# ClashLuke/LocAtE

Measured on AMD Instinct MI355X. Metric: images/sec (G+D step) 64x64 bs=64, higher is better.
Workload: dtype f32 (contractions fp32-faithful on the matrix cores: 2 x scaled fp16 operand pieces / 3 MFMAs per slice where the operand's largest magnitude comes with it, else 3 x bf16 pieces / 6 MFMAs; fp32 accumulate); 1 GPU; LocAtE G+D step, 64x64 RGB, batch 64 per GPU (the fp32 variant - the reference's own precision - of BASELINE.json configs[1]: 64x64 RGB bs 64), self/feature attention at 16x16 and 64x64, random-init weights; global_batch=64, image_size=64, parallelism=dp1, launch=hipGraph replay, G-step generator pass on a second stream

## Files before the change

include/locate_hip.h:

```cpp
#ifndef LOCATE_HIP_H
#define LOCATE_HIP_H
#include <stddef.h>
#include <stdint.h>
#ifdef __cplusplus
extern "C" {
#endif

const char* locate_last_error(void);
int locate_abi_version(void);
int locate_device_info(char* arch_name, int name_len, int* cu_count, int* wave_size);

int locate_roottanh_fwd(const float* x, float* y, int64_t n, void* absmax , void* stream);
int locate_absmax_words(void);
int locate_roottanh_bwd(const float* x, const float* gy, float* gx, int64_t n, int accumulate, void* absmax, void* stream);
int locate_absmax(const float* x, int64_t n, void* absmax, void* stream);
int locate_act_cat_rows_fwd(const float* latent, const float* pre, float* out, int rows, int z, int w, void* stream);
int locate_act_rows_bwd(const float* pre, const float* g, int64_t g_row_stride, const float* g_add, float* gpre, int rows, int w,
                        void* stream);
int locate_add3(const float* a, int64_t a_bs, const float* b, int64_t b_bs, const float* c, int64_t c_bs, float* out, int batch,
                int64_t per, void* stream);
int locate_tanh_fwd(const float* x, float* y, int64_t n, void* stream);
int locate_tanh_bwd(const float* y, const float* gy, float* gx, int64_t n, void* stream);

size_t locate_norm_stats_workspace_bytes(void);
// ... 32 lines not shown
int locate_pool2_upsample2x_fwd(const float* x, float* y, int64_t planes, int H, int W, void* stream);
int locate_pool2_upsample2x_bwd(const float* gy, float* gx, int64_t planes, int H, int W, int accumulate, void* stream);
int locate_avgpool2_fwd(const float* x, float* y, int64_t planes, int H, int W, void* stream);
int locate_avgpool2_bwd(const float* gy, float* gx, int64_t planes, int H, int W, int accumulate, void* stream);
int locate_feature_pool_fwd(const float* x, float* y, int64_t n_out, int r, void* stream);
int locate_feature_pool_bwd(const float* gy, float* gx, int64_t n_out, int r, int accumulate, void* stream);
int locate_copy_channels(const float* src, float* dst, int B, int C, int hw, int64_t src_batch_stride,
                         int64_t dst_batch_stride, int accumulate, void* stream);

size_t locate_sn_workspace_bytes(int h, int wd);
int locate_sn_power_iter(const float* w, float* u, float* v, float* sigma, float* wv, int h, int wd, void* workspace,
                         void* stream);
size_t locate_sn_table_record_bytes(void);
int locate_sn_power_iter_batched(const void* table, int n_layers, int max_h, int max_wd, void* stream);
int locate_sn_weight_bwd(const double* inner_partial, int n_partial, const float* u, const float* v, const float* sigma,
                         const float* wv, float* gw, float* du, float* dsigma_out, int h, int wd, void* stream);
size_t locate_sn_group_workspace_bytes(void);
int locate_sn_weight_bwd_grouped(const float* gy, int64_t gy_bs, const float* y, int64_t y_bs, const float* bias, int groups,
                                 int Bg, int M, int plane, const float* sigma_tab, int sigma_stride, const float* u,
                                 const float* v, const float* wv, int64_t wv_stride, float* gw, float* du,
                                 float* dsigma_total_out, int h, int wd, void* workspace, void* stream);
int locate_sn_dv_batched(const void* table, int n_layers, int max_h, int max_wd, void* stream);

size_t locate_conv_panel_bytes(const int* geom, int adjoint);
int locate_conv_pack_panel(const int* geom, int adjoint, const float* w, float* panel, void* stream);
size_t locate_conv_pack_job_bytes(void);
int locate_conv_pack_job(const int* geom, int adjoint, const float* w, float* panel, int block_start, void* job_out,
                         int* blocks_out, int direct, const void* weight_absmax);
int locate_conv_pack_panels(const void* jobs, int n_jobs, int total_blocks, int any_f16, int passes, void* stream);
int locate_conv_pack_job_is_direct(const void* job);
int locate_conv_pack_job_is_window(const void* job);
int locate_conv_win_ok(const int* geom, int adjoint_fmt, int64_t x_bs, const void* x);
size_t locate_conv_win_workspace_bytes(const int* geom, int adjoint_fmt);
size_t locate_conv_fwd_workspace_bytes(const int* geom);
size_t locate_conv_counter_bytes(void);
int locate_conv_fwd(const int* geom, const float* x, int64_t x_bs, const float* panel, const float* scale,
                    int scale_group_batch, int scale_stride, const float* bias, float* y, int64_t y_bs, void* workspace,
                    void* counters, int precision, const void* x_absmax, const void* act_epilogue, void* stream);
size_t locate_conv_dgrad_workspace_bytes(const int* geom);
int locate_conv_dgrad(const int* geom, const float* gy, int64_t gy_bs, const float* panel, const float* scale,
                      int scale_group_batch, int scale_stride, const float* bias, float* gx, int64_t gx_bs, void* workspace,
                      void* counters, int precision, const void* gy_absmax, const void* act_epilogue, void* stream);
size_t locate_conv_wgrad_workspace_bytes(const int* geom);
int locate_conv_wgrad_partials(const int* geom);
int locate_conv_wgrad(const int* geom, const float* x, int64_t x_bs, const float* gy, int64_t gy_bs, float* gw,
                      const float* w_ref, const float* inv_scale, int scale_group_batch, int scale_stride,
                      double* inner_partial, void* workspace, int precision, const void* x_absmax, const void* gy_absmax,
                      void* deferred_reduce, void* stream);
int locate_conv_wgrad_group_partials(const int* geom, int groups);
size_t locate_conv_wgrad_group_workspace_bytes(const int* geom, int groups);
size_t locate_slab_reduce_record_bytes(void);
int locate_slab_reduce_max(void);
int locate_slab_reduce_record_blocks(const void* record);
int locate_slab_reduce_batch(const void* records, int n, void* stream);

size_t locate_wgrad_batch_record_bytes(void);
int locate_wgrad_batch_max(void);
int locate_wgrad_batch_record(const int* geom, const float* x, int64_t x_bs, const float* gy, int64_t gy_bs, float* gw,
                              const float* w_ref, const float* inv_scale, int scale_group_batch, int scale_stride,
                              double* inner_partial, void* record);
int locate_wgrad_batch(const void* records, int n, void* stream);

int locate_dwconv_fwd(const int* geom, const float* x, int64_t x_bs, const float* w, const float* scale, int scale_group_batch,
                      int scale_stride, float* y, int64_t y_bs, void* stream);
int locate_dwconv_dgrad(const int* geom, const float* gy, int64_t gy_bs, const float* w, const float* scale,
                        int scale_group_batch, int scale_stride, float* gx, int64_t gx_bs, void* stream);
// ... 82 lines not shown
```

locate_amd/_lib.py:

```python
import ctypes
import os

import torch

_HERE = os.path.dirname(os.path.abspath(__file__))
LIB_PATH = os.path.join(_HERE, "csrc", "liblocate_hip_dbg.so" if os.environ.get("LOCATE_HIP_DEBUG_LIBRARY") == "1"
                        else "liblocate_hip.so")

c_p = ctypes.c_void_p
c_i = ctypes.c_int
c_i64 = ctypes.c_int64
c_f = ctypes.c_float
c_d = ctypes.c_double
c_sz = ctypes.c_size_t
c_ip = ctypes.POINTER(ctypes.c_int)

PROTOTYPES = {
    "locate_last_error": (ctypes.c_char_p, []),
    "locate_abi_version": (c_i, []),
    "locate_device_info": (c_i, [ctypes.c_char_p, c_i, c_ip, c_ip]),
    "locate_roottanh_fwd": (c_i, [c_p, c_p, c_i64, c_p, c_p]),
    "locate_roottanh_bwd": (c_i, [c_p, c_p, c_p, c_i64, c_i, c_p, c_p]),
    "locate_act_cat_rows_fwd": (c_i, [c_p, c_p, c_p, c_i, c_i, c_i, c_p]),
    "locate_act_rows_bwd": (c_i, [c_p, c_p, c_i64, c_p, c_p, c_i, c_i, c_p]),
# ... 20 lines not shown
    "locate_gate_fwd": (c_i, [c_p, c_p, c_i, c_p, c_p, c_i64, c_i, c_p]),
    "locate_gate_fwd_stats": (c_i, [c_p, c_p, c_i, c_p, c_p, c_i64, c_i, c_i, c_p, c_p]),
    "locate_gate_bwd_workspace_bytes": (c_sz, [c_i64]),
    "locate_gate_bwd": (c_i, [c_p, c_p, c_i, c_p, c_p, c_p, c_p, c_p, c_i64, c_i, c_p, c_i, c_p, c_p]),
    "locate_softmax_fwd": (c_i, [c_p, c_p, c_i64, c_i, c_p]),
    "locate_softmax_bwd": (c_i, [c_p, c_p, c_p, c_i64, c_i, c_p]),
    "locate_upsample2x_fwd": (c_i, [c_p, c_p, c_i64, c_i, c_i, c_p]),
    "locate_upsample2x_bwd": (c_i, [c_p, c_p, c_i64, c_i, c_i, c_p]),
    "locate_pool2_upsample2x_fwd": (c_i, [c_p, c_p, c_i64, c_i, c_i, c_p]),
    "locate_pool2_upsample2x_bwd": (c_i, [c_p, c_p, c_i64, c_i, c_i, c_i, c_p]),
    "locate_avgpool2_fwd": (c_i, [c_p, c_p, c_i64, c_i, c_i, c_p]),
    "locate_avgpool2_bwd": (c_i, [c_p, c_p, c_i64, c_i, c_i, c_i, c_p]),
    "locate_feature_pool_fwd": (c_i, [c_p, c_p, c_i64, c_i, c_p]),
    "locate_feature_pool_bwd": (c_i, [c_p, c_p, c_i64, c_i, c_i, c_p]),
    "locate_copy_channels": (c_i, [c_p, c_p, c_i, c_i, c_i, c_i64, c_i64, c_i, c_p]),
    "locate_sn_workspace_bytes": (c_sz, [c_i, c_i]),
    "locate_sn_power_iter": (c_i, [c_p, c_p, c_p, c_p, c_p, c_i, c_i, c_p, c_p]),
    "locate_sn_table_record_bytes": (c_sz, []),
    "locate_sn_power_iter_batched": (c_i, [c_p, c_i, c_i, c_i, c_p]),
    "locate_sn_weight_bwd": (c_i, [c_p, c_i, c_p, c_p, c_p, c_p, c_p, c_p, c_p, c_i, c_i, c_p]),
    "locate_sn_group_workspace_bytes": (c_sz, []),
    "locate_sn_weight_bwd_grouped": (c_i, [c_p, c_i64, c_p, c_i64, c_p, c_i, c_i, c_i, c_i, c_p, c_i, c_p, c_p, c_p, c_i64, c_p,
                                           c_p, c_p, c_i, c_i, c_p, c_p]),
    "locate_sn_dv_batched": (c_i, [c_p, c_i, c_i, c_i, c_p]),
    "locate_conv_panel_bytes": (c_sz, [c_ip, c_i]),
    "locate_conv_pack_panel": (c_i, [c_ip, c_i, c_p, c_p, c_p]),
    "locate_conv_pack_job_bytes": (c_sz, []),
    "locate_conv_pack_job": (c_i, [c_ip, c_i, c_p, c_p, c_i, c_p, c_ip, c_i, c_p]),
    "locate_conv_pack_panels": (c_i, [c_p, c_i, c_i, c_i, c_i, c_p]),
    "locate_conv_pack_job_is_direct": (c_i, [c_p]),
    "locate_conv_pack_job_is_window": (c_i, [c_p]),
    "locate_conv_win_ok": (c_i, [c_ip, c_i, c_i64, c_p]),
    "locate_conv_win_workspace_bytes": (c_sz, [c_ip, c_i]),
    "locate_conv_fwd_workspace_bytes": (c_sz, [c_ip]),
    "locate_conv_counter_bytes": (c_sz, []),
    "locate_conv_fwd": (c_i, [c_ip, c_p, c_i64, c_p, c_p, c_i, c_i, c_p, c_p, c_i64, c_p, c_p, c_i, c_p, c_p, c_p]),
    "locate_conv_dgrad_workspace_bytes": (c_sz, [c_ip]),
    "locate_conv_dgrad": (c_i, [c_ip, c_p, c_i64, c_p, c_p, c_i, c_i, c_p, c_p, c_i64, c_p, c_p, c_i, c_p, c_p, c_p]),
    "locate_conv_wgrad_workspace_bytes": (c_sz, [c_ip]),
    "locate_conv_wgrad_partials": (c_i, [c_ip]),
    "locate_conv_wgrad": (c_i, [c_ip, c_p, c_i64, c_p, c_i64, c_p, c_p, c_p, c_i, c_i, c_p, c_p, c_i, c_p, c_p, c_p, c_p]),
    "locate_conv_wgrad_group_partials": (c_i, [c_ip, c_i]),
    "locate_conv_wgrad_group_workspace_bytes": (c_sz, [c_ip, c_i]),
    "locate_slab_reduce_record_bytes": (c_sz, []),
    "locate_slab_reduce_max": (c_i, []),
    "locate_slab_reduce_record_blocks": (c_i, [c_p]),
    "locate_slab_reduce_batch": (c_i, [c_p, c_i, c_p]),
    "locate_dwconv_fwd": (c_i, [c_ip, c_p, c_i64, c_p, c_p, c_i, c_i, c_p, c_i64, c_p]),
    "locate_dwconv_dgrad": (c_i, [c_ip, c_p, c_i64, c_p, c_p, c_i, c_i, c_p, c_i64, c_p]),
    "locate_dwconv_wgrad_workspace_bytes": (c_sz, [c_ip]),
    "locate_dwconv_wgrad_partials": (c_i, [c_ip]),
    "locate_dwconv_wgrad": (c_i, [c_ip, c_p, c_i64, c_p, c_i64, c_p, c_p, c_p, c_i, c_i, c_p, c_p, c_p]),
    "locate_groupdot_fwd": (c_i, [c_p, c_i64, c_p, c_p, c_i, c_i, c_p, c_i, c_i, c_i, c_p]),
    "locate_groupdot_dgrad": (c_i, [c_p, c_p, c_p, c_i, c_i, c_p, c_i64, c_i, c_i, c_i, c_p]),
    "locate_groupdot_wgrad_partials": (c_i, [c_i, c_i]),
    "locate_groupdot_wgrad": (c_i, [c_p, c_i64, c_p, c_p, c_p, c_p, c_i, c_i, c_p, c_i, c_i, c_i, c_p]),
    "locate_fin_record_bytes": (c_sz, []),
    "locate_fin_sn_dot_partials": (c_i, [c_i, c_i, c_i]),
    "locate_fin_sn_dots": (c_i, [c_p, c_i, c_p]),
    "locate_fin_sn_rank1": (c_i, [c_p, c_i, c_p]),
    "locate_fin_sums": (c_i, [c_p, c_i, c_p]),
    "locate_fin_channel_slices": (c_i, [c_i, c_i, c_i]),
    "locate_fin_channel_sums": (c_i, [c_p, c_i, c_p]),
    "locate_gate_bwd_partials": (c_i, [c_i64, c_i]),
    "locate_multi_copy_record_bytes": (c_sz, []),
    "locate_multi_copy_chunk_elems": (c_i, []),
# ... 84 lines not shown
```

locate_amd/csrc/conv.hip:

```cpp
#include "igemm.h"

template <int WGM, int WGN, int TM, int TN>
__global__ void __launch_bounds__(256) conv_igemm_kernel(const IgParams p) {
    constexpr int BK = IG_BK;
    constexpr int BM = WGM * TM * 32;
    constexpr int BN = WGN * TN * 32;
    constexpr int KPT = BK * BN / 256;
    constexpr int A_F4 = BK * BM / 4;
    constexpr int A_PT = (A_F4 + 255) / 256;
    static_assert(WGM * WGN == 4, "four waves");
    static_assert(BN % 64 == 0 && KPT == 8, "one 8-row group of the offset table per thread and step");
    static_assert(BK <= IG_TAIL, "panel tail shorter than the prefetch distance (one stage beyond the last)");

    __shared__ __attribute__((aligned(16))) float As[2][BK][BM];
    __shared__ __attribute__((aligned(16))) float Bs[2][BK][BN];

    int bx, by, bz;
    xcd_tile(bx, by, bz, p.tile_nphase);
    const int zphase = bz / p.ksplit, zsplit = bz - zphase * p.ksplit;
    const IgPhase& ph = p.ph[zphase];
    const int N = p.B * ph.QH * ph.QW;
    const int n0 = bx * BN;
    const int m0 = by * BM;
    if (n0 >= N) return;
// ... 764 lines not shown
    *lo = first; *n = last - first + 1;
}

static void phase_taps(int parity, int pad, int K, int s, int* k0, int* d0, int* T) {
    *k0 = (parity + pad) % s;
    *d0 = (parity + pad - *k0) / s;
    *T = *k0 < K ? (K - *k0 + s - 1) / s : 0;
}

static int tap_dmin(const PackArgs& a) {
    int best = 0;
    for (int th = 0; th < a.TH; ++th)
        for (int tw = 0; tw < a.TW; ++tw) {
            const int d = (a.dy0 + a.dys * th) * a.gW + a.dx0 + a.dxs * tw;
            if (d < best) best = d;
        }
    return best;
}

static void phase_finish(IgPhase& ph, const PackArgs& pa, float* panel_base) {
    ph.wp = panel_base;
    ph.koff = reinterpret_cast<const int*>(panel_base + (size_t)pa.rows * pa.ld);
    ph.ktap = reinterpret_cast<const unsigned char*>(ph.koff + pa.rows);
    ph.w3 = reinterpret_cast<const uint4*>(panel_base + panel_split_offset(pa.rows, pa.ld) + (pa.fmt ? PANEL_HDR : 0));
    ph.a_absmax = pa.fmt ? reinterpret_cast<const unsigned*>(panel_base + panel_split_offset(pa.rows, pa.ld)) : nullptr;
    ph.w3_plane = (long long)(pa.rows / 8) * pa.ld;
    ph.dmin = pa.dmin;
    ph.K = pa.K; ph.Kpad = pa.rows - IG_TAIL; ph.ld = pa.ld;
    ph.TW = pa.TW > 0 ? pa.TW : 1; ph.tw_magic = (65536 + ph.TW - 1) / ph.TW;
    ph.dy0 = pa.dy0; ph.dys = pa.dys; ph.dx0 = pa.dx0; ph.dxs = pa.dxs;
}

#define WIN_LDS_BUDGET (128 * 1024)
static bool win_finish(IgParams& p, PackBatch& batch, int fmt, float* panel, size_t* off_out) {
    if (path_disabled("win") || p.nphase < 1 || p.C < 16 || (p.C & 7)) return false;
    bool any1 = false;
    for (int i = 0; i < p.nphase; ++i) {
        if (p.ph[i].T < 1) return false;
        any1 = any1 || p.ph[i].T == 1;
    }
    if (any1 && (p.nphase > 1 || p.istride != 1 || p.ostep != 1 || p.ph[0].dy0 != 0 || p.ph[0].dx0 != 0 || p.H != p.OH || p.W != p.OW)) return false;
    if (any1) {
        const long long HW = (long long)p.H * p.W;
        if (HW < 2 || (HW & (HW - 1)) != 0) return false;
        int bn1 = 128;
        if (knob_int("LOCATE_WIN_BM", 0) > 0 && p.M % knob_int("LOCATE_WIN_BM", 0) == 0) bn1 = win_pick_bn(knob_int("LOCATE_WIN_BM", 0));
        if (knob_int("LOCATE_WIN_BN", 0) > 0) bn1 = knob_int("LOCATE_WIN_BN", 0);
        const int Wc = HW >= bn1 ? bn1 : (int)HW;
        p.W = p.OW = Wc; p.H = p.OH = (int)(HW / Wc);
        p.ph[0].QW = Wc; p.ph[0].QH = p.H;
        p.ph[0].TW = 1; p.ph[0].tw_magic = 65536;
    }
    if ((p.W & 1) || (((long long)p.H * p.W) & 1)) return false;
    int bm = win_pick_bm(p.M), bn = win_pick_bn(bm);
    if (any1) {
        const long long N1 = (long long)p.B * p.H * p.W;
        bn = 128;
        bm = ((N1 + 127) / 128) * ((p.M + 63) / 64) >= 256 ? 64 : 32;
        if (round_up(p.M, 64) != round_up(p.M, 32)) bm = 32;
    }
    {
        const int fbm = knob_int("LOCATE_WIN_BM", 0), fbn = knob_int("LOCATE_WIN_BN", 0);
        if (fbm > 0 && p.M % fbm == 0) { bm = fbm; bn = win_pick_bn(bm); }
        if (fbn > 0) bn = fbn;
    }
    const int C8G = (p.C + 7) / 8;
// ... 30 lines not shown
        if (items > 2ll * 256 * ph.win_NG) return false;
        if (items > 256ll * ph.win_NG) bpt = 2;
        for (int t = 0; t < 32; ++t) {
            int c = 0;
            if (t < T) {
                const int th = t / ph.TW, tw = t - th * ph.TW;
                const int dy = ph.dy0 + ph.dys * th, dx = ph.dx0 + ph.dxs * tw;
                c = dy * p.W + (p.istride == 2 ? (dx & 1) * (p.W / 2) + (dx >> 1) : dx);
            }
            ph.tapc[t] = c;
        }
        const int C8Gp = T == 1 ? round_up(C8G, U) : C8G;
        pa.win = 1; pa.Tp = ph.win_Tp; pa.urows = C8Gp * ph.win_Tp + WIN_TAIL_UNITS;
        pa.out = panel ? panel + off : nullptr;
        ph.wp = nullptr; ph.koff = nullptr; ph.ktap = nullptr;
        ph.a_absmax = (fmt && pa.out) ? reinterpret_cast<const unsigned*>(pa.out) : nullptr;
        ph.w3 = pa.out ? reinterpret_cast<const uint4*>(pa.out + PANEL_HDR) : nullptr;
        ph.w3_plane = (long long)pa.urows * pa.ld;
        ph.Kpad = C8Gp * ph.win_Tp * 8;
        pa.wmax = (fmt && pa.out) ? reinterpret_cast<const unsigned*>(pa.out) : nullptr;
        pa.wmax_single = 1;
        off += win_panel_floats(pa.urows, pa.ld, fmt);
    }
    if (p.istride == 2 && (p.W & (p.W - 1))) return false;
    int ngm = 1;
    for (int i = 0; i < p.nphase; ++i) ngm = p.ph[i].win_NG > ngm ? p.ph[i].win_NG : ngm;
    const size_t lds = ((size_t)2 * NP * U * bm + (size_t)2 * NP * (any1 ? U : 1) * slotsp) * 16 + (size_t)ngm * bpt * 256 * 8;
    if (lds > WIN_LDS_BUDGET) return false;
    if (any1)
        for (int t = 0; t < 32; ++t) p.ph[0].tapc[t] = t < U ? t * slotsp : 0;
    p.win = 1; p.win_U = U; p.win_slotsp = slotsp; p.win_bm = bm; p.win_bn = bn;
    *off_out = off;
    return true;
}

static int conv_plan(const ConvGeom& g, int adjoint_fmt, const float* w, float* panel, IgParams& p, int* nmax_out,
                     size_t* panel_floats_out, bool pack, hipStream_t st, PackBatch* batch_out = nullptr) {
    const int adjoint = adjoint_fmt & 1, fmt = (adjoint_fmt & 8) ? 2 : ((adjoint_fmt >> 1) & 1);
    size_t off = 0;
    int nmax = 0;
    p.nphase = 0;
    PackBatch batch;
    if (!adjoint) {
        p.B = g.B; p.C = g.C; p.H = g.H; p.W = g.W; p.M = g.M; p.OH = g.OH; p.OW = g.OW;
        p.istride = g.stride; p.ostep = 1; p.nphase = 1;
        PackArgs pa;
        pa.w = w; pa.out = panel;
        pa.M = g.M; pa.C = g.C; pa.KH = g.KH; pa.KW = g.KW; pa.mode = 0;
        pa.s = 1;
        useful_taps(g.H, g.OH, g.KH, g.stride, g.pad_h, &pa.kh0, &pa.TH);
        useful_taps(g.W, g.OW, g.KW, g.stride, g.pad_w, &pa.kw0, &pa.TW);
        pa.K = g.C * pa.TH * pa.TW; pa.rows = round_up(pa.K, IG_KPAD) + IG_TAIL; pa.ld = round_up(g.M, 32);
        pa.gHW = g.H * g.W; pa.gW = g.W; pa.dy0 = pa.kh0 - g.pad_h; pa.dys = 1; pa.dx0 = pa.kw0 - g.pad_w; pa.dxs = 1;
        pa.dmin = tap_dmin(pa);
        pa.fmt = fmt; pa.wmax = nullptr; pa.direct = 0; pa.keep_f32 = 1;
        pa.win = 0; pa.Tp = 0; pa.urows = 0; pa.wmax_single = 0;
        batch.ph[0] = pa;
        IgPhase& ph = p.ph[0];
        phase_finish(ph, pa, panel);
        ph.T = pa.TH * pa.TW;
        ph.oy0 = ph.ox0 = 0; ph.QH = g.OH; ph.QW = g.OW;
        off = panel_floats(pa.rows, pa.ld, fmt);
        nmax = g.B * g.OH * g.OW;
    } else {
        p.B = g.B; p.C = g.M; p.H = g.OH; p.W = g.OW; p.M = g.C; p.OH = g.H; p.OW = g.W;
        p.istride = 1; p.ostep = g.stride;
// ... 145 lines not shown
        p.mul_pre = static_cast<const float*>(epi->mul_pre); p.mul_bs = epi->mul_bs;
    }
    if (epi && (epi->act_out || epi->mul_pre)) p.out_absmax = static_cast<unsigned*>(epi->out_absmax);
    return launch_igemm(p, nmax, ws, counters, st, who);
}

static size_t igemm_ws_bytes(const int* geom, int adjoint) {
    IgParams p;
    p.precision = 0;
    int nmax = 0;
    if (conv_plan(make_geom(geom), adjoint, nullptr, nullptr, p, &nmax, nullptr, false, nullptr)) return 0;
    return (p.nphase > 0 ? slab_floats(p, nmax) : 0) * sizeof(float);
}

LOCATE_API int locate_conv_win_ok(const int* geom, int adjoint_fmt, int64_t x_bs, const void* x) {
    const ConvGeom g = make_geom(geom);
    if (geom_check(g, "locate_conv_win_ok")) return 0;
    if ((x_bs & 1) || (reinterpret_cast<uintptr_t>(x) & 7)) return 0;
    IgParams p;
    p.precision = 0;
    int nmax = 0;
    if (conv_plan(g, adjoint_fmt & 1, nullptr, nullptr, p, &nmax, nullptr, false, nullptr) || p.nphase < 1) return 0;
    p.in = static_cast<const float*>(x); p.out = nullptr; p.in_bs = x_bs; p.out_bs = 2;
    if (skinny_ok(p)) return 0;
    {
        const IgPhase& ph = p.ph[0];
        if (p.nphase == 1 && ph.T == 1 && p.istride == 1 && p.ostep == 1 && p.H == p.OH && p.W == p.OW && ph.K <= 64 && p.M <= 64 &&
            (long long)p.B * p.H * p.W >= 131072 && !path_disabled("pointwise")) return 0;
    }
    if (conv_plan(g, (adjoint_fmt & 3) | 4, nullptr, nullptr, p, &nmax, nullptr, false, nullptr) || !p.win) return 0;
    bool taps4 = p.nphase == 4;
    for (int i = 0; i < p.nphase; ++i) taps4 = taps4 && p.ph[i].T == 4;
    const bool best = p.M >= 128 && ((p.nphase == 1 && p.ph[0].T == 1 && p.C >= 384) || (taps4 && p.C >= 512));
    return best ? 1 : 2;
}
LOCATE_API size_t locate_conv_win_workspace_bytes(const int* geom, int adjoint_fmt) {
    IgParams p;
    p.precision = (adjoint_fmt & 2) ? 2 : 0;
    int nmax = 0;
    if (conv_plan(make_geom(geom), (adjoint_fmt & 3) | 4, nullptr, nullptr, p, &nmax, nullptr, false, nullptr) || !p.win) return 0;
    return win_slab_floats(p, nmax) * sizeof(float);
}

LOCATE_API size_t locate_conv_fwd_workspace_bytes(const int* geom) { return igemm_ws_bytes(geom, 0); }
LOCATE_API size_t locate_conv_dgrad_workspace_bytes(const int* geom) { return igemm_ws_bytes(geom, 1); }

LOCATE_API size_t locate_conv_counter_bytes(void) { return IG_MAX_COUNTERS * sizeof(unsigned); }

LOCATE_API int locate_conv_fwd(const int* geom, const float* x, int64_t x_bs, const float* panel, const float* scale,
                               int scale_group_batch, int scale_stride, const float* bias, float* y, int64_t y_bs,
                               void* workspace, void* counters, int precision, const void* x_absmax, const void* act_epilogue,
                               void* stream) {
    const ConvGeom g = make_geom(geom);
    if (int e = geom_check(g, "locate_conv_fwd")) return e;
    LOCATE_REQUIRE(x && panel && y, "locate_conv_fwd: null pointer");
    return run_igemm(g, 0, x, x_bs, panel, scale, scale_group_batch, scale_stride, bias, y, y_bs, static_cast<float*>(workspace),
                     static_cast<unsigned*>(counters), precision, static_cast<const unsigned*>(x_absmax), as_stream(stream), "locate_conv_fwd",
                     static_cast<const LocateActEpilogue*>(act_epilogue));
}

LOCATE_API int locate_conv_dgrad(const int* geom, const float* gy, int64_t gy_bs, const float* panel, const float* scale,
                                 int scale_group_batch, int scale_stride, const float* bias, float* gx, int64_t gx_bs,
                                 void* workspace, void* counters, int precision, const void* gy_absmax, const void* act_epilogue,
                                 void* stream) {
    const ConvGeom g = make_geom(geom);
    if (int e = geom_check(g, "locate_conv_dgrad")) return e;
    LOCATE_REQUIRE(gy && panel && gx, "locate_conv_dgrad: null pointer");
// ... 5 lines not shown
```

locate_amd/csrc/convwin.hip:

```cpp
#include "igemm.h"

typedef unsigned u32x2 __attribute__((ext_vector_type(2)));
typedef int i32x2 __attribute__((ext_vector_type(2)));
typedef int i32x4 __attribute__((ext_vector_type(4)));

template <int WGM, int WGN, int TM, int TN, int NP, int SL, int BPT>
__global__ void __launch_bounds__(256, 2) conv_win_kernel(const IgParams p) {
    constexpr int NT = 256, NW = 4, U = 2 * SL;
    constexpr int BM = WGM * TM * 32;
    constexpr int BN = WGN * TN * 32;
    static_assert(WGM * WGN == NW && (BN == 128 || BN == 256), "four waves on a 128- or 256-column tile");
    constexpr int A_CH = U * BM;
    constexpr int A_PT = (A_CH + NT - 1) / NT;
    constexpr int A_U4 = 2 * NP * A_CH;
    static_assert(2 * U <= WIN_TAIL_UNITS, "panel tail shorter than the prefetch distance");

    extern __shared__ uint4 smem[];

    int bx, by, bz;
    xcd_tile(bx, by, bz, p.tile_nphase);
    const int zphase = bz / p.ksplit, zsplit = bz - zphase * p.ksplit;
    const IgPhase& ph = p.ph[zphase];
    const int QHW = ph.QH * ph.QW;
    const int N = p.B * QHW;
// ... 356 lines not shown
        const unsigned zstride = (unsigned)ntiles * tile_bytes;
#pragma unroll
        for (int i = 0; i < TM; ++i)
#pragma unroll
            for (int j = 0; j < TN; ++j)
#pragma unroll
                for (int r = 0; r < 16; ++r) acc[i][j][r] = 0.0f;
        constexpr int HB = 4, ZB = 4;
#pragma unroll
        for (int h0 = 0; h0 < FR; h0 += HB) {
            for (int z0 = 0; z0 < p.ksplit; z0 += ZB) {
                u32x4 v[ZB][HB];
#pragma unroll
                for (int zz = 0; zz < ZB; ++zz)
#pragma unroll
                    for (int f = 0; f < HB; ++f)
                        v[zz][f] = __builtin_amdgcn_raw_buffer_load_b128(srs, (int)(t0 + (unsigned)(z0 + zz) * zstride + (unsigned)((h0 + f) * NT * 16)), 0, 16);
#pragma unroll
                for (int zz = 0; zz < ZB; ++zz)
#pragma unroll
                    for (int f = 0; f < HB; ++f) {
                        const int gg = h0 + f, i = gg / (TN * 4), j = (gg / 4) % TN, q = gg % 4;
#pragma unroll
                        for (int e = 0; e < 4; ++e) acc[i][j][4 * q + e] += __uint_as_float(v[zz][f][e]);
                    }
            }
        }
        __syncthreads();
        combined = true;
    }
    igemm_epilogue<WGM, WGN, TM, TN>(p, ph, acc, col_scale, N, n0, m0, combined ? 0 : zsplit, wm, wn, lane, stage, p.ksplit > 1 && !combined);
}

struct WinSplit {
    int ksplit, combine, gx, gy;
    size_t slab_floats;
};

static int win_nwin(const IgParams& p) {
    const int C8G = (p.C + 7) / 8;
    return p.ph[0].win_Tp == 1 ? (C8G + p.win_U - 1) / p.win_U : C8G;
}

static WinSplit win_split_plan(const IgParams& p, int nmax, bool have_counters) {
    WinSplit sp;
    const int bm = p.win_bm;
    sp.gx = (nmax + p.win_bn - 1) / p.win_bn;
    sp.gy = (p.M + bm - 1) / bm;
    const long long tiles = (long long)sp.gx * sp.gy * p.nphase;
    const int nwin = win_nwin(p);
    int ks = 1;
    if (tiles < 384) {
        long long want = (512 + tiles - 1) / tiles;
        const int max_split = nwin / 2 > 0 ? nwin / 2 : 1;
        if (want > max_split) want = max_split;
        if (want > 16) want = 16;
        ks = want < 1 ? 1 : (int)want;
        const int per = (nwin + ks - 1) / ks;
        ks = (nwin + per - 1) / per;
    }
    sp.ksplit = ks;
    const long long tile_floats = (long long)bm * p.win_bn;
    const long long legacy = ks > 1 ? (long long)ks * p.B * p.M * p.OH * p.OW : 0;
    const long long fused = ks > 1 ? (long long)ks * tiles * tile_floats : 0;
    sp.combine = have_counters && ks > 1 && (long long)ks * tile_floats * 4 <= (512 << 10) && tiles <= 1024 && fused * 4 < (1ll << 31);
    sp.slab_floats = (size_t)(sp.combine ? fused : legacy);
    return sp;
}

size_t win_slab_floats(const IgParams& p, int nmax) {
    const size_t a = win_split_plan(p, nmax, false).slab_floats, b = win_split_plan(p, nmax, true).slab_floats;
    return a > b ? a : b;
}

template <int WGM, int WGN, int TM, int TN, int NP, int SL>
static void win_launch_bpt(const IgParams& p, dim3 grid, size_t lds, int bpt, hipStream_t st) {
    if (bpt <= 1) {
        auto k = conv_win_kernel<WGM, WGN, TM, TN, NP, SL, 1>;
        static bool enabled = false;
        if (!enabled) { (void)hipFuncSetAttribute(reinterpret_cast<const void*>(k), hipFuncAttributeMaxDynamicSharedMemorySize, 160 * 1024); enabled = true; }
        k<<<grid, 256, lds, st>>>(p);
    } else {
        auto k = conv_win_kernel<WGM, WGN, TM, TN, NP, SL, 2>;
        static bool enabled = false;
        if (!enabled) { (void)hipFuncSetAttribute(reinterpret_cast<const void*>(k), hipFuncAttributeMaxDynamicSharedMemorySize, 160 * 1024); enabled = true; }
        k<<<grid, 256, lds, st>>>(p);
    }
}

template <int NP, int SL>
static void win_launch_bm(const IgParams& p, dim3 grid, size_t lds, int bpt, hipStream_t st) {
    const int bm = p.win_bm;
    if (p.win_bn == 128 && bm == 96) win_launch_bpt<1, 4, 3, 1, NP, SL>(p, grid, lds, bpt, st);
    else if (p.win_bn == 128 && bm == 64) win_launch_bpt<1, 4, 2, 1, NP, SL>(p, grid, lds, bpt, st);
    else if (p.win_bn == 128 && bm == 32) win_launch_bpt<1, 4, 1, 1, NP, SL>(p, grid, lds, bpt, st);
    else if (bm == 192) win_launch_bpt<2, 2, 3, 2, NP, SL>(p, grid, lds, bpt, st);
    else if (bm == 128) win_launch_bpt<2, 2, 2, 2, NP, SL>(p, grid, lds, bpt, st);
    else if (bm == 96) win_launch_bpt<1, 4, 3, 2, NP, SL>(p, grid, lds, bpt, st);
    else if (bm == 64) win_launch_bpt<1, 4, 2, 2, NP, SL>(p, grid, lds, bpt, st);
    else win_launch_bpt<1, 4, 1, 2, NP, SL>(p, grid, lds, bpt, st);
}

template <int NP>
static void win_launch_sl(const IgParams& p, dim3 grid, size_t lds, int bpt, hipStream_t st) {
    if (p.win_U == 2) win_launch_bm<NP, 1>(p, grid, lds, bpt, st);
    else win_launch_bm<NP, 2>(p, grid, lds, bpt, st);
}

int launch_win_igemm(IgParams& p, int nmax, void* slab_ws, unsigned* counters, hipStream_t st, const char* who) {
    const WinSplit sp = win_split_plan(p, nmax, counters != nullptr);
    p.ksplit = sp.ksplit;
    p.combine = sp.combine;
    p.counters = counters;
    p.slab = static_cast<float*>(slab_ws);
    p.slab_stride = (long long)p.B * p.M * p.OH * p.OW;
    LOCATE_REQUIRE(p.ksplit == 1 || slab_ws, "%s: split-K needs a workspace", who);
    p.win_dbg = knob_int("LOCATE_WIN_DBG", 0);
    const int NP = p.precision == 2 ? 2 : (p.precision == 1 ? 1 : 3);
    const int U = p.win_U, bm = p.win_bm;
    const bool single = p.ph[0].win_Tp == 1;
    for (int i = 0; i < p.nphase; ++i)
        LOCATE_REQUIRE(round_up(p.M, bm) <= p.ph[i].ld, "%s: tile height %d does not divide the panel width %d", who, bm, p.ph[i].ld);
    int bpt = 1;
    for (int i = 0; i < p.nphase; ++i) {
        const IgPhase& ph = p.ph[i];
        const long long items = (long long)(single ? U : 1) * (ph.win_NI * ph.win_WR * p.W / 2);
        const int need = (int)((items + 256ll * ph.win_NG - 1) / (256ll * ph.win_NG));
        if (need > bpt) bpt = need;
    }
    LOCATE_REQUIRE(bpt <= 2, "%s: window of %d items per thread", who, bpt);
    int ng_max = 1;
    for (int i = 0; i < p.nphase; ++i) ng_max = p.ph[i].win_NG > ng_max ? p.ph[i].win_NG : ng_max;
    size_t lds = ((size_t)2 * NP * U * bm + (size_t)2 * NP * (single ? U : 1) * p.win_slotsp) * 16 + (size_t)ng_max * bpt * 256 * 8;
    const size_t epi = (size_t)4 * 32 * 33 * 4 + 64;
    if (lds < epi) lds = epi;
    LOCATE_REQUIRE(lds <= 160 * 1024, "%s: window images of %zu bytes exceed the LDS", who, lds);
    dim3 grid(sp.gx, sp.gy, p.nphase * p.ksplit);
    if (NP == 2) win_launch_sl<2>(p, grid, lds, bpt, st);
    else if (NP == 3) win_launch_sl<3>(p, grid, lds, bpt, st);
    else win_launch_sl<1>(p, grid, lds, bpt, st);
    LOCATE_LAUNCH_CHECK(who);
    if (p.ksplit > 1 && !p.combine) {
// ... 7 lines not shown
```

locate_amd/csrc/igemm.h:

```cpp
#pragma once
#include "common.h"
#include <cstdlib>
#include <cstring>
#include <stdlib.h>
#include <type_traits>

#ifdef LOCATE_DEBUG_KNOBS
static bool path_disabled(const char* name) {
    static const char* env = getenv("LOCATE_DISABLE");
    return env != nullptr && strstr(env, name) != nullptr;
}
static int knob_int(const char* name, int fallback) {
    const char* v = getenv(name);
    return v != nullptr ? atoi(v) : fallback;
}
#else
static constexpr bool path_disabled(const char*) { return false; }
static constexpr int knob_int(const char*, int fallback) { return fallback; }
#endif

typedef float f32x16 __attribute__((ext_vector_type(16)));

#define IG_BK 16
#define IG_KPAD 32
// ... 454 lines not shown
    return __builtin_bit_cast(float, __builtin_amdgcn_raw_buffer_load_b32(g.rsrc, (int)vo, soff, 0));
}

typedef int i32x8 __attribute__((ext_vector_type(8)));
typedef unsigned u32x4 __attribute__((ext_vector_type(4)));


__device__ __forceinline__ int fastdiv(int n, unsigned mul, int s1, int s2) {
    const unsigned t = __umulhi((unsigned)n, mul);
    return (int)((t + (((unsigned)n - t) >> s1)) >> s2);
}
static void fastdiv_make(unsigned d, unsigned* mul, int* s1, int* s2) {
    if (d <= 1) { *mul = 0; *s1 = 0; *s2 = 0; return; }
    int l = 0;
    while ((1ull << l) < d) ++l;
    *mul = (unsigned)(((1ull << 32) * ((1ull << l) - d)) / d + 1);
    *s1 = 1; *s2 = l - 1;
}

#define WIN_TAIL_UNITS 16

static inline int win_pick_bm(int M) { return (M >= 192 && M % 192 == 0) ? 192 : pick_bm(M); }
static inline int win_pick_bn(int bm) { return bm >= 128 ? 128 : 256; }
static inline int win_pick_sl(const int* X, int nx) {
    long long real = 0, padded = 0;
    for (int i = 0; i < nx; ++i) { real += X[i]; padded += (X[i] + 3) / 4 * 4; }
    return (padded - real) * 100 <= 15 * real ? 2 : 1;
}

static inline int win_pack_cs(int KK) { return KK <= 4 ? 64 : (KK <= 16 ? 32 : 16); }
static inline __host__ __device__ int win_pack_rg(int KK) { return KK == 1 ? 64 : 16; }
static inline size_t win_panel_floats(int urows, int ld, int fmt) { return PANEL_HDR + (size_t)(fmt ? 2 : 3) * urows * ld * 4; }

int launch_win_igemm(IgParams& p, int nmax, void* slab_ws, unsigned* counters, hipStream_t st, const char* who);
void launch_fp8_igemm(const IgParams& p, dim3 grid, int bm, hipStream_t st);
size_t win_slab_floats(const IgParams& p, int nmax);
void launch_slab_reduce(const IgParams& p, hipStream_t st);
```

Baseline: 7278 images/sec.

## Add persistent LDS-resident-weight window conv kernel for small-M large-pixel convs

Adds a persistent implicit-GEMM convolution kernel for the window path. The whole split-precision weight panel stays resident in LDS (up to 160 KB), and each CU walks a contiguous range of 256-pixel tiles, double-buffering input windows through registers with buffer loads. It is used for single-phase, stride-1 convs with M<=64 and tile-aligned outputs, and replaces the split-K and slab path, so those cases need no slab workspace. The goal is to stop re-streaming weights for every tile on the many-pixel, few-channel convs at 64x64. The cost is one block per CU with large LDS use, which limits occupancy, plus a new code path with its own epilogue that must match the existing fused-activation behaviour.

```diff
diff --git a/include/locate_hip.h b/include/locate_hip.h
--- a/include/locate_hip.h
+++ b/include/locate_hip.h
@@ -88,6 +88,7 @@
 int locate_conv_pack_job_is_window(const void* job);
 int locate_conv_win_ok(const int* geom, int adjoint_fmt, int64_t x_bs, const void* x);
 size_t locate_conv_win_workspace_bytes(const int* geom, int adjoint_fmt);
+int locate_conv_win_resident(const int* geom, int adjoint_fmt);
 size_t locate_conv_fwd_workspace_bytes(const int* geom);
 size_t locate_conv_counter_bytes(void);
 int locate_conv_fwd(const int* geom, const float* x, int64_t x_bs, const float* panel, const float* scale,
diff --git a/locate_amd/_lib.py b/locate_amd/_lib.py
--- a/locate_amd/_lib.py
+++ b/locate_amd/_lib.py
@@ -76,6 +76,7 @@
     "locate_conv_pack_job_is_window": (c_i, [c_p]),
     "locate_conv_win_ok": (c_i, [c_ip, c_i, c_i64, c_p]),
     "locate_conv_win_workspace_bytes": (c_sz, [c_ip, c_i]),
+    "locate_conv_win_resident": (c_i, [c_ip, c_i]),
     "locate_conv_fwd_workspace_bytes": (c_sz, [c_ip]),
     "locate_conv_counter_bytes": (c_sz, []),
     "locate_conv_fwd": (c_i, [c_ip, c_p, c_i64, c_p, c_p, c_i, c_i, c_p, c_p, c_i64, c_p, c_p, c_i, c_p, c_p, c_p]),
diff --git a/locate_amd/csrc/conv.hip b/locate_amd/csrc/conv.hip
--- a/locate_amd/csrc/conv.hip
+++ b/locate_amd/csrc/conv.hip
@@ -820,6 +820,7 @@
 }
 
 #define WIN_LDS_BUDGET (128 * 1024)
+#define WIN_RESIDENT_MIN_PIXELS 131072ll
 static bool win_finish(IgParams& p, PackBatch& batch, int fmt, float* panel, size_t* off_out) {
     if (path_disabled("win") || p.nphase < 1 || p.C < 16 || (p.C & 7)) return false;
     bool any1 = false;
@@ -916,6 +917,17 @@
     p.win = 1; p.win_U = U; p.win_slotsp = slotsp; p.win_bm = bm; p.win_bn = bn;
     *off_out = off;
     return true;
+}
+
+bool win_resident_ok(const IgParams& p, int NP) {
+    if (!p.win || path_disabled("resident")) return false;
+    if (p.nphase != 1 || p.istride != 1 || p.ostep != 1 || p.M > 64) return false;
+    const IgPhase& ph = p.ph[0];
+    if (ph.T <= 1 || ph.oy0 != 0 || ph.ox0 != 0) return false;
+    if (p.win_bn != 256 || ph.win_NI != 1 || (ph.QH * ph.QW) % 256 != 0 || 256 % ph.QW != 0) return false;
+    if (ph.QH != p.OH || ph.QW != p.OW) return false;
+    if (ph.win_WR * p.W > 4 * 256) return false;
+    return win_resident_lds(p, NP) <= WIN_RESIDENT_LDS;
 }
 
 static int conv_plan(const ConvGeom& g, int adjoint_fmt, const float* w, float* panel, IgParams& p, int* nmax_out,
@@ -1127,7 +1139,22 @@
     bool taps4 = p.nphase == 4;
     for (int i = 0; i < p.nphase; ++i) taps4 = taps4 && p.ph[i].T == 4;
     const bool best = p.M >= 128 && ((p.nphase == 1 && p.ph[0].T == 1 && p.C >= 384) || (taps4 && p.C >= 512));
-    return best ? 1 : 2;
+    const bool resident = win_resident_ok(p, (adjoint_fmt & 2) ? 2 : 3) && (long long)nmax >= WIN_RESIDENT_MIN_PIXELS;
+    return (best || resident) ? 1 : 2;
+}
+LOCATE_API int locate_conv_win_resident(const int* geom, int adjoint_fmt) {
+    const ConvGeom g = make_geom(geom);
+    if (geom_check(g, "locate_conv_win_resident")) return 0;
+    IgParams p;
+    p.precision = (adjoint_fmt & 2) ? 2 : 0;
+    int nmax = 0;
+    {
+        if (conv_plan(g, adjoint_fmt & 1, nullptr, nullptr, p, &nmax, nullptr, false, nullptr) || p.nphase < 1) return 0;
+        p.in = nullptr; p.out = nullptr; p.in_bs = 2; p.out_bs = 2;
+        if (skinny_ok(p)) return 0;
+    }
+    if (conv_plan(g, (adjoint_fmt & 3) | 4, nullptr, nullptr, p, &nmax, nullptr, false, nullptr) || !p.win) return 0;
+    return win_resident_ok(p, (adjoint_fmt & 2) ? 2 : 3) ? 1 : 0;
 }
 LOCATE_API size_t locate_conv_win_workspace_bytes(const int* geom, int adjoint_fmt) {
     IgParams p;
diff --git a/locate_amd/csrc/convwin.hip b/locate_amd/csrc/convwin.hip
--- a/locate_amd/csrc/convwin.hip
+++ b/locate_amd/csrc/convwin.hip
@@ -412,6 +412,381 @@
     igemm_epilogue<WGM, WGN, TM, TN>(p, ph, acc, col_scale, N, n0, m0, combined ? 0 : zsplit, wm, wn, lane, stage, p.ksplit > 1 && !combined);
 }
 
+typedef float f32x4 __attribute__((ext_vector_type(4)));
+
+template <int NP, int MT>
+__global__ void __launch_bounds__(256, 1) conv_win_resident_kernel(const IgParams p, const int ntiles) {
+    constexpr int NT = 256, TNW = 4, MC = MT * 16, BPT = 2;
+    extern __shared__ uint4 smem[];
+
+    const IgPhase& ph = p.ph[0];
+    const int tid = threadIdx.x, lane = tid & 63, wid = tid >> 6;
+    const int l16 = lane & 15, kq = lane >> 4;
+    const int T = ph.T, Tp = ph.win_Tp, NS = (T + 3) >> 2;
+    const int TH = T / ph.TW;
+    const int C8G = p.C >> 3;
+    const int NUL = win_resident_units(p);
+    const int SP = p.win_slotsp;
+    const int W = p.W, HW = p.H * p.W, QW = ph.QW, QHW = ph.QH * ph.QW;
+    const int WRW = ph.win_WR * W;
+    const int dyA = ph.dy0, dyB = ph.dy0 + ph.dys * (TH - 1);
+    const int dymin = dyA < dyB ? dyA : dyB;
+
+    const int t_lo = (int)((long long)blockIdx.x * ntiles / (int)gridDim.x);
+    const int t_hi = (int)((long long)(blockIdx.x + 1) * ntiles / (int)gridDim.x);
+    if (t_lo >= t_hi) return;
+
+    uint4* const Ap = smem;
+    uint4* const Bw = smem + NP * NUL * MC;
+    int* const tapt = reinterpret_cast<int*>(Bw + 2 * NP * SP);
+#ifdef LOCATE_DEBUG_KNOBS
+    const int dbg = p.win_dbg;
+#endif
+
+    const __amdgpu_buffer_rsrc_t rsrc = __builtin_amdgcn_make_buffer_rsrc(const_cast<float*>(p.in), 0, (int)p.in_bytes, 0x00020000);
+    const unsigned HW4 = 4u * (unsigned)HW;
+    const bool two = WRW > 2 * NT;
+    u32x2 breg[BPT][8];
+    int ltile = t_lo, lg = 0;
+    unsigned l_base = 0, l_wso = 0;
+    int l_lim = 0;
+    auto next_window = [&]() {
+        const int n0 = ltile * 256;
+        const int b = n0 / QHW, qy0 = (n0 - b * QHW) / QW;
+        int iy_lo = qy0 + dymin;
+        if (iy_lo < 0) iy_lo = 0;
+        l_base = (unsigned)(4 * ((long long)b * p.in_bs + (long long)iy_lo * W));
+        int lim = HW - iy_lo * W;
+        if (lim > WRW) lim = WRW;
+        l_lim = ltile < t_hi ? lim : 0;
+        l_wso = (unsigned)(lg * 8) * HW4;
+        if (++lg == C8G) { lg = 0; ++ltile; }
+    };
+    auto issue_item = [&](auto ic) {
+        constexpr int i = decltype(ic)::value;
+        const int s2 = 2 * (tid + i * NT);
+        const unsigned voff = s2 < l_lim ? l_base + 4u * (unsigned)s2 : 0x80000000u;
+#pragma unroll
+        for (int e = 0; e < 8; ++e)
+            breg[i][e] = __builtin_bit_cast(u32x2, __builtin_amdgcn_raw_buffer_load_b64(rsrc, (int)voff, (int)(l_wso + (unsigned)e * HW4), 0));
+    };
+    float b_scale = 1.0f, a_unscale = 1.0f, b_unscale = 1.0f;
+    if constexpr (NP == 2) {
+        const int kb_ = f16_scale_exp(absmax_read(p.b_absmax));
+        const int ka_ = f16_scale_exp(__builtin_amdgcn_readfirstlane(*ph.a_absmax));
+        b_scale = pow2f(kb_);
+        unscale_pair(ka_, kb_, a_unscale, b_unscale);
+    }
+    auto store_item = [&](auto ic, int buf) {
+        constexpr int i = decltype(ic)::value;
+        uint4* Bs = Bw + buf * NP * SP;
+        const int s2 = 2 * (tid + i * NT);
+        const bool on = s2 < WRW;
+#pragma unroll
+        for (int v = 0; v < 2; ++v) {
+            float f[8];
+#pragma unroll
+            for (int e = 0; e < 8; ++e) f[e] = __uint_as_float(v == 0 ? breg[i][e].x : breg[i][e].y);
+            uint4* dst = Bs + (on ? s2 + v : SP - 2);
+            if constexpr (NP == 2) {
+                uint4 h, l;
+                split2_f16x8(f, b_scale, h, l);
+                dst[0] = h;
+                dst[SP] = l;
+            } else if constexpr (NP == 3) {
+                uint4 h, m, l;
+                split3_trunc_x8(f, h, m, l);
+                dst[0] = h;
+                dst[SP] = m;
+                dst[2 * SP] = l;
+            } else {
+                bf16x8 h;
+#pragma unroll
+                for (int e = 0; e < 8; ++e) h[e] = (__bf16)f[e];
+                dst[0] = *reinterpret_cast<uint4*>(&h);
+            }
+        }
+    };
+    using I0 = std::integral_constant<int, 0>;
+    using I1 = std::integral_constant<int, 1>;
+
+    next_window();
+    issue_item(I0{});
+    if (two) issue_item(I1{});
+    {
+        constexpr int PB = 12;
+        const int total = NUL * MC;
+        for (int e0 = 0; e0 < total; e0 += PB * NT) {
+            uint4 v[NP][PB];
+#pragma unroll
+            for (int q = 0; q < NP; ++q)
+#pragma unroll
+                for (int i = 0; i < PB; ++i) {
+                    const int e = e0 + i * NT + tid;
+                    const int ec = e < total ? e : 0;
+                    const int u = ec / MC, m = ec - u * MC;
+                    v[q][i] = ph.w3[(long long)q * ph.w3_plane + (long long)u * ph.ld + m];
+                }
+#pragma unroll
+            for (int q = 0; q < NP; ++q)
+#pragma unroll
+                for (int i = 0; i < PB; ++i) {
+                    const int e = e0 + i * NT + tid;
+                    if (e < total) Ap[q * total + e] = v[q][i];
+                }
+        }
+    }
+    if (tid < 2 * NP) Bw[tid * SP + SP - 1] = make_uint4(0u, 0u, 0u, 0u);
+    if (tid < 32) tapt[tid] = ph.tapc[tid];
+    store_item(I0{}, 0);
+    if (two) store_item(I1{}, 0);
+    next_window();
+    issue_item(I0{});
+    if (two) issue_item(I1{});
+
+    int prow[TNW], qx[TNW];
+    unsigned colin[TNW];
+#pragma unroll
+    for (int j = 0; j < TNW; ++j) {
+        const int po = wid * 64 + j * 16 + l16;
+        prow[j] = po / QW;
+        qx[j] = po - prow[j] * QW;
+        unsigned c = 0;
+        for (int tw = 0; tw < ph.TW; ++tw) c |= ((unsigned)(qx[j] + ph.dx0 + ph.dxs * tw) < (unsigned)W ? 1u : 0u) << tw;
+        colin[j] = c;
+    }
+    float bias_v[MT][4];
+#pragma unroll
+    for (int i = 0; i < MT; ++i)
+#pragma unroll
+        for (int r = 0; r < 4; ++r) {
+            const int m = i * 16 + 4 * kq + r;
+            const bool use = p.bias != nullptr && m < p.M;
+            const float* bp = use ? p.bias + m : p.in;
+            bias_v[i][r] = use ? *bp : 0.0f;
+        }
+    const bool fused = p.act_out != nullptr || p.mul_pre != nullptr;
+    float am = 0.0f;
+    __syncthreads();
+    constexpr int MAXS = 7;
+    int toffs[MAXS];
+#pragma unroll
+    for (int s = 0; s < MAXS; ++s) toffs[s] = tapt[4 * s + kq];
+
+    using frag_t = typename std::conditional<NP == 2, f16x8, bf16x8>::type;
+    constexpr int PROD = NP == 3 ? 6 : (NP == 2 ? 3 : 1);
+    constexpr int NMF = MT * TNW * PROD;
+    int kk = 0;
+    for (int tile = t_lo; tile < t_hi; ++tile) {
+        const int n0 = tile * 256;
+        const int b = n0 / QHW, q0 = n0 - b * QHW, qy0 = q0 / QW;
+        int iy_lo = qy0 + dymin;
+        if (iy_lo < 0) iy_lo = 0;
+        const float cs = p.scale ? p.scale[(p.scale_bg ? b / p.scale_bg : 0) * p.scale_stride] : 1.0f;
+        int lbase[TNW];
+        unsigned outs[TNW];
+#pragma unroll
+        for (int j = 0; j < TNW; ++j) {
+            const int iy0 = qy0 + prow[j];
+            unsigned inside = 0;
+            for (int th = 0; th < TH; ++th)
+                if ((unsigned)(iy0 + ph.dy0 + ph.dys * th) < (unsigned)p.H) inside |= colin[j] << (th * ph.TW);
+            outs[j] = ~inside;
+            lbase[j] = (iy0 - iy_lo) * W + qx[j];
+        }
+        f32x4 acc[MT][TNW];
+#pragma unroll
+        for (int i = 0; i < MT; ++i)
+#pragma unroll
+            for (int j = 0; j < TNW; ++j)
+#pragma unroll
+                for (int r = 0; r < 4; ++r) acc[i][j][r] = 0.0f;
+
+        for (int g = 0; g < C8G; ++g) {
+            const uint4* Bsb = Bw + (kk & 1) * NP * SP;
+            const uint4* Asb = Ap + g * Tp * MC;
+            frag_t fa[2][MT][NP], fb[2][TNW][NP];
+            auto load_frags = [&](int s, int set) {
+                const int t = 4 * s + kq;
+#pragma unroll
+                for (int i = 0; i < MT; ++i)
+#pragma unroll
+                    for (int q = 0; q < NP; ++q) fa[set][i][q] = *reinterpret_cast<const frag_t*>(&Asb[q * NUL * MC + t * MC + i * 16 + l16]);
+#pragma unroll
+                for (int j = 0; j < TNW; ++j) {
+                    const bool out = (outs[j] >> t) & 1u;
+                    const int addr = out ? SP - 1 : lbase[j] + toffs[s];
+#pragma unroll
+                    for (int q = 0; q < NP; ++q) fb[set][j][q] = *reinterpret_cast<const frag_t*>(&Bsb[q * SP + addr]);
+                }
+            };
+            auto mfmas = [&](int set) {
+#ifdef LOCATE_DEBUG_KNOBS
+                if (dbg & 1) return;
+#endif
+#pragma unroll
+                for (int i = 0; i < MT; ++i)
+#pragma unroll
+                    for (int j = 0; j < TNW; ++j) {
+                        frag_t (&a)[NP] = fa[set][i];
+                        frag_t (&bb)[NP] = fb[set][j];
+                        if constexpr (NP == 2) {
+                            acc[i][j] = __builtin_amdgcn_mfma_f32_16x16x32_f16(a[1], bb[0], acc[i][j], 0, 0, 0);
+                            acc[i][j] = __builtin_amdgcn_mfma_f32_16x16x32_f16(a[0], bb[1], acc[i][j], 0, 0, 0);
+                            acc[i][j] = __builtin_amdgcn_mfma_f32_16x16x32_f16(a[0], bb[0], acc[i][j], 0, 0, 0);
+                        } else if constexpr (NP == 3) {
+                            acc[i][j] = __builtin_amdgcn_mfma_f32_16x16x32_bf16(a[NP - 1], bb[0], acc[i][j], 0, 0, 0);
+                            acc[i][j] = __builtin_amdgcn_mfma_f32_16x16x32_bf16(a[0], bb[NP - 1], acc[i][j], 0, 0, 0);
+                            acc[i][j] = __builtin_amdgcn_mfma_f32_16x16x32_bf16(a[NP - 2], bb[NP - 2], acc[i][j], 0, 0, 0);
+                            acc[i][j] = __builtin_amdgcn_mfma_f32_16x16x32_bf16(a[NP - 2], bb[0], acc[i][j], 0, 0, 0);
+                            acc[i][j] = __builtin_amdgcn_mfma_f32_16x16x32_bf16(a[0], bb[NP - 2], acc[i][j], 0, 0, 0);
+                            acc[i][j] = __builtin_amdgcn_mfma_f32_16x16x32_bf16(a[0], bb[0], acc[i][j], 0, 0, 0);
+                        } else {
+                            acc[i][j] = __builtin_amdgcn_mfma_f32_16x16x32_bf16(a[0], bb[0], acc[i][j], 0, 0, 0);
+                        }
+                    }
+            };
+            load_frags(0, 0);
+#ifdef LOCATE_DEBUG_KNOBS
+            const bool moves = !(dbg & 2);
+#else
+            constexpr bool moves = true;
+#endif
+            if (moves) next_window();
+            if (moves && two) {
+                store_item(I1{}, (kk & 1) ^ 1);
+                issue_item(I1{});
+            }
+            if (1 < NS) load_frags(1, 1);
+            if (moves) {
+                store_item(I0{}, (kk & 1) ^ 1);
+                issue_item(I0{});
+            }
+            mfmas(0);
+#pragma unroll
+            for (int k = 0; k < NMF; ++k) {
+                __builtin_amdgcn_sched_group_barrier(0x008, 1, 0);
+                __builtin_amdgcn_sched_group_barrier(0x002, 4, 0);
+                __builtin_amdgcn_sched_group_barrier(0x200, 1, 0);
+                __builtin_amdgcn_sched_group_barrier(0x020, 1, 0);
+            }
+#pragma unroll
+            for (int s = 1; s < MAXS; ++s) {
+                if (s < NS) {
+                    if (s + 1 < NS) load_frags(s + 1 < MAXS ? s + 1 : 0, (s + 1) & 1);
+                    mfmas(s & 1);
+                }
+            }
+            ++kk;
+            __syncthreads();
+        }
+
+        const long long plane = (long long)p.OH * p.OW;
+        const long long pix0 = (long long)q0 + wid * 64 + l16;
+        float* const obase = p.out + (long long)b * p.out_bs + pix0;
+#pragma unroll
+        for (int i = 0; i < MT; ++i) {
+            float v[TNW][4];
+#pragma unroll
+            for (int j = 0; j < TNW; ++j)
+#pragma unroll
+                for (int r = 0; r < 4; ++r) {
+                    float a = acc[i][j][r];
+                    if constexpr (NP == 2) a = (a * a_unscale) * b_unscale;
+                    v[j][r] = fmaf(a, cs, bias_v[i][r]);
+                }
+            if (!fused) {
+#pragma unroll
+                for (int j = 0; j < TNW; ++j)
+#pragma unroll
+                    for (int r = 0; r < 4; ++r) {
+                        const int m = i * 16 + 4 * kq + r;
+                        if (m < p.M) obase[(long long)m * plane + j * 16] = v[j][r];
+                    }
+            } else if (p.mul_pre != nullptr) {
+                const float* pre = p.mul_pre + (long long)b * p.mul_bs + pix0;
+                float z[TNW][4];
+#pragma unroll
+                for (int j = 0; j < TNW; ++j)
+#pragma unroll
+                    for (int r = 0; r < 4; ++r) {
+                        const int m = i * 16 + 4 * kq + r;
+                        z[j][r] = m < p.M ? pre[(long long)m * plane + j * 16] : 0.0f;
+                    }
+#pragma unroll
+                for (int j = 0; j < TNW; ++j)
+#pragma unroll
+                    for (int r = 0; r < 4; ++r) {
+                        const int m = i * 16 + 4 * kq + r;
+                        const float o = roottanh_grad_f(z[j][r], v[j][r]);
+                        if (m < p.M) { obase[(long long)m * plane + j * 16] = o; am = fmaxf(am, fabsf(o)); }
+                    }
+                __builtin_amdgcn_sched_barrier(0);
+            } else {
+                float* const abase = p.act_out + (long long)b * p.act_bs + pix0;
+#pragma unroll
+                for (int j = 0; j < TNW; ++j)
+#pragma unroll
+                    for (int r = 0; r < 4; ++r) {
+                        const int m = i * 16 + 4 * kq + r;
+                        const float a = roottanh_f(v[j][r]);
+                        if (m < p.M) { obase[(long long)m * plane + j * 16] = v[j][r]; abase[(long long)m * plane + j * 16] = a; am = fmaxf(am, fabsf(a)); }
+                    }
+                __builtin_amdgcn_sched_barrier(0);
+            }
+        }
+    }
+    if (fused && p.out_absmax != nullptr) absmax_publish_wave(am, p.out_absmax);
+}
+
+static int device_cus() {
+    static int cus[64];
+    int dev = 0;
+    if (hipGetDevice(&dev) != hipSuccess) return 0;
+    int n = 0;
+    if (dev >= 0 && dev < 64 && cus[dev] > 0) return cus[dev];
+    if (hipDeviceGetAttribute(&n, hipDeviceAttributeMultiprocessorCount, dev) != hipSuccess) return 0;
+    if (dev >= 0 && dev < 64) cus[dev] = n;
+    return n;
+}
+
+template <int NP, int MT>
+static void win_resident_launch(const IgParams& p, int ntiles, int grid, size_t lds, hipStream_t st) {
+    auto k = conv_win_resident_kernel<NP, MT>;
+    static bool enabled[64];
+    int dev = 0;
+    (void)hipGetDevice(&dev);
+    if (dev < 0 || dev >= 64 || !enabled[dev]) {
+        (void)hipFuncSetAttribute(reinterpret_cast<const void*>(k), hipFuncAttributeMaxDynamicSharedMemorySize, WIN_RESIDENT_LDS);
+        if (dev >= 0 && dev < 64) enabled[dev] = true;
+    }
+    k<<<grid, 256, lds, st>>>(p, ntiles);
+}
+
+template <int NP>
+static void win_resident_mt(const IgParams& p, int ntiles, int grid, size_t lds, hipStream_t st) {
+    const int mt = (p.M + 15) / 16;
+    if (mt == 1) win_resident_launch<NP, 1>(p, ntiles, grid, lds, st);
+    else if (mt == 2) win_resident_launch<NP, 2>(p, ntiles, grid, lds, st);
+    else if (mt == 3) win_resident_launch<NP, 3>(p, ntiles, grid, lds, st);
+    else win_resident_launch<NP, 4>(p, ntiles, grid, lds, st);
+}
+
+static int launch_win_resident(IgParams& p, int NP, hipStream_t st, const char* who) {
+    const int ntiles = (int)((long long)p.B * p.ph[0].QH * p.ph[0].QW / 256);
+    const int cus = device_cus();
+    LOCATE_REQUIRE(cus > 0, "%s: cannot read the device's CU count", who);
+    const int grid = ntiles < cus ? ntiles : cus;
+    const size_t lds = win_resident_lds(p, NP);
+    p.ksplit = 1;
+    p.combine = 0;
+    if (NP == 2) win_resident_mt<2>(p, ntiles, grid, lds, st);
+    else if (NP == 3) win_resident_mt<3>(p, ntiles, grid, lds, st);
+    else win_resident_mt<1>(p, ntiles, grid, lds, st);
+    LOCATE_LAUNCH_CHECK(who);
+    return LOCATE_OK;
+}
+
 struct WinSplit {
     int ksplit, combine, gx, gy;
     size_t slab_floats;
@@ -449,6 +824,7 @@
 }
 
 size_t win_slab_floats(const IgParams& p, int nmax) {
+    if (win_resident_ok(p, p.precision == 2 ? 2 : (p.precision == 1 ? 1 : 3))) return 0;
     const size_t a = win_split_plan(p, nmax, false).slab_floats, b = win_split_plan(p, nmax, true).slab_floats;
     return a > b ? a : b;
 }
@@ -488,6 +864,13 @@
 }
 
 int launch_win_igemm(IgParams& p, int nmax, void* slab_ws, unsigned* counters, hipStream_t st, const char* who) {
+    {
+        const int np = p.precision == 2 ? 2 : (p.precision == 1 ? 1 : 3);
+        if (win_resident_ok(p, np)) {
+            p.win_dbg = knob_int("LOCATE_WIN_DBG", 0);
+            return launch_win_resident(p, np, st, who);
+        }
+    }
     const WinSplit sp = win_split_plan(p, nmax, counters != nullptr);
     p.ksplit = sp.ksplit;
     p.combine = sp.combine;
diff --git a/locate_amd/csrc/igemm.h b/locate_amd/csrc/igemm.h
--- a/locate_amd/csrc/igemm.h
+++ b/locate_amd/csrc/igemm.h
@@ -510,6 +510,16 @@
 static inline __host__ __device__ int win_pack_rg(int KK) { return KK == 1 ? 64 : 16; }
 static inline size_t win_panel_floats(int urows, int ld, int fmt) { return PANEL_HDR + (size_t)(fmt ? 2 : 3) * urows * ld * 4; }
 
+#define WIN_RESIDENT_LDS (160 * 1024)
+static inline __host__ __device__ int win_resident_units(const IgParams& p) {
+    return ((p.C >> 3) - 1) * p.ph[0].win_Tp + ((p.ph[0].T + 3) >> 2) * 4;
+}
+static inline size_t win_resident_lds(const IgParams& p, int NP) {
+    const size_t mc = (size_t)((p.M + 15) / 16) * 16;
+    return (mc * win_resident_units(p) * NP + (size_t)2 * NP * p.win_slotsp) * 16 + 32 * 4;
+}
+bool win_resident_ok(const IgParams& p, int NP);
+
 int launch_win_igemm(IgParams& p, int nmax, void* slab_ws, unsigned* counters, hipStream_t st, const char* who);
 void launch_fp8_igemm(const IgParams& p, dim3 grid, int bm, hipStream_t st);
 size_t win_slab_floats(const IgParams& p, int nmax);
```

Result: no change. 7267 images/sec (-0.1%).
